# BananaFalls/LDPC-NeuralNetwork-Decoder

Hardware: AMD Instinct MI355X
Metric: codewords/s at fixed SNR (BG2, 10 iters) (higher is better)
Workload: dtype f32

## Files before the change

ldpc-neuralnetwork-decoder_amd/csrc/flood_dev.hpp:

```cpp
#pragma once
#include <algorithm>
#include <cmath>
#include <cstdint>
#include <cstdlib>

#include <utility>

#include "common.hpp"
#include "graph.hpp"

namespace ldpc {

constexpr int kPartRow = 8;
constexpr int ES_P1 = 3, ES_P2 = 4;

struct EsWs {
    uint64_t *words;
    uint32_t *valid;
    int nvw;
    uint64_t *cand;
    int32_t *twg;
    int32_t *ctl;
    uint64_t *staged;
};
// ... 95 lines not shown
typedef float f32x2 __attribute__((ext_vector_type(2)));

struct MinSumStats {
    int nz = 0;
    bool neg = false;
    float m1 = INFINITY, m2 = INFINITY;
    int i1 = -1;
    __device__ __forceinline__ void add(int e, float x) {
        const float a = fabsf(x);
        nz += is_zero_sign(x);
        neg ^= (x < 0.0f);
        const bool lt1 = a < m1, lt2 = a < m2;
        m2 = lt1 ? m1 : (lt2 ? a : m2);
        i1 = lt1 ? e : i1;
        m1 = lt1 ? a : m1;
    }
    __device__ __forceinline__ float c2v(int e, float x, float alpha) const {
        const float m = (e == i1) ? m2 : m1;
        const int zex = nz - (int)is_zero_sign(x);
        const float s = zex > 0 ? 0.0f : ((neg ^ (x < 0.0f)) ? -1.0f : 1.0f);
        return s * (alpha * m);
    }
};

template <int DC, int CAP>
__device__ __forceinline__ uint32_t sign_parity_n(const float (&v)[CAP]) {
    static_assert(DC <= CAP, "row longer than its buffer");
    uint32_t p = __float_as_uint(v[0]);
#pragma unroll
    for (int e = 1; e + 1 < DC; e += 2)
        asm("v_bitop3_b32 %0, %1, %2, %3 bitop3:0x96" : "=v"(p) : "v"(p), "v"(v[e]), "v"(v[e + 1]));
    if constexpr (DC % 2 == 0) p ^= __float_as_uint(v[DC - 1]);
    return p;
}

__device__ __forceinline__ float opaque_sf(float v) {
    asm volatile("" : "+s"(v));
    return v;
}
__device__ __forceinline__ uint32_t opaque_vu(uint32_t v) {
    asm volatile("" : "+v"(v));
    return v;
}
__device__ __forceinline__ float opaque_vf(float v) {
    asm volatile("" : "+v"(v));
    return v;
}
__device__ __forceinline__ void two_min_step(float &m1, float &m2, float x, float ninf) {
    m2 = __builtin_amdgcn_fmed3f(m1, fabsf(x), m2);
    m1 = __builtin_amdgcn_fmed3f(m1, fabsf(x), ninf);
}

__device__ __forceinline__ float vmin(float a, float b) { return __builtin_elementwise_minimum(a, b); }
__device__ __forceinline__ float vmax(float a, float b) { return __builtin_elementwise_maximum(a, b); }
template <int DC, int CAP>
__device__ __forceinline__ void two_smallest(const float (&v)[CAP], float &m1, float &m2, float ninf) {
    static_assert(DC <= CAP, "row longer than its buffer");
    if constexpr (DC == 1) {
        m1 = fabsf(v[0]);
    } else if constexpr (DC == 2) {
        m1 = vmin(fabsf(v[0]), fabsf(v[1]));
        m2 = vmax(fabsf(v[0]), fabsf(v[1]));
    } else {
        m1 = vmin(vmin(fabsf(v[0]), fabsf(v[1])), fabsf(v[2]));
        m2 = __builtin_amdgcn_fmed3f(fabsf(v[0]), fabsf(v[1]), fabsf(v[2]));
        constexpr int NT = (DC - 3) / 3;
        sfor<NT>([&](auto q) {
            constexpr int B0 = 3 + 3 * decltype(q)::value;
            const float a = fabsf(v[B0]), b = fabsf(v[B0 + 1]), c = fabsf(v[B0 + 2]);
            const float t1 = vmin(vmin(a, b), c), t2 = __builtin_amdgcn_fmed3f(a, b, c);
            m2 = vmin(vmin(vmax(m1, t1), m2), t2);
            m1 = vmin(m1, t1);
        });
        sfor<DC - 3 - 3 * NT>([&](auto q) { two_min_step(m1, m2, v[3 + 3 * NT + decltype(q)::value], ninf); });
    }
}

__device__ __forceinline__ uint64_t cmp_eq_abs(float x, float m) {
    uint64_t k;
    asm volatile("v_cmp_eq_f32_e64 %0, |%1|, %2" : "=s"(k) : "v"(x), "v"(m));
    return k;
}
__device__ __forceinline__ uint32_t cndmask(uint32_t if0, uint32_t if1, uint64_t k) {
    uint32_t r;
    asm volatile("v_cndmask_b32_e64 %0, %1, %2, %3" : "=v"(r) : "v"(if0), "v"(if1), "s"(k));
    return r;
}

struct MinSumFast {
    float m1 = INFINITY, m2 = INFINITY;
    uint32_t par = 0;
    bool special = false;
    __device__ __forceinline__ void add(float x) {
        const float a = fabsf(x);
        special |= is_zero_sign(x);
        m2 = __builtin_amdgcn_fmed3f(m1, a, m2);
        asm("v_min_f32 %0, %1, |%2|" : "=v"(m1) : "v"(m1), "v"(x));
    }
    __device__ __forceinline__ float c2v(float x, uint32_t s1, uint32_t s2) const {
        const uint32_t sel = fabsf(x) == m1 ? s2 : s1;
        return __uint_as_float((__float_as_uint(x) & 0x80000000u) ^ sel);
    }
    __device__ __forceinline__ void sel_words(float alpha, uint32_t &s1, uint32_t &s2) const {
        const uint32_t ps = par & 0x80000000u;
        s1 = __float_as_uint(fabsf(alpha * m1)) | ps;
        s2 = __float_as_uint(fabsf(alpha * m2)) | ps;
    }
};

__device__ __forceinline__ float tanh_half(float v) {
    const float y = v * 0.5f;
    const float a = fabsf(y), z = y * y;
    float p = fmaf(-5.70498872745e-3f, z, 2.06390887954e-2f);
    p = fmaf(p, z, -5.37397155531e-2f);
    p = fmaf(p, z, 1.33314422036e-1f);
    p = fmaf(p, z, -3.33332819422e-1f);
    const float small = fmaf(p * z, a, a);
    const float e = __builtin_amdgcn_exp2f(a * 2.88539008177792681f);
    const float big = fmaf(-2.0f, __builtin_amdgcn_rcpf(e + 1.0f), 1.0f);
    return copysignf(a < 0.625f ? small : big, y);
}
__device__ __forceinline__ float two_atanh(float x) {
    const float z = x * x;
    float p = fmaf(1.81740078349e-1f, z, 8.24370301058e-2f);
    p = fmaf(p, z, 1.46691431730e-1f);
    p = fmaf(p, z, 1.99782164500e-1f);
    p = fmaf(p, z, 3.33337300303e-1f);
    const float small = 2.0f * fmaf(p * z, x, x);
    const float r = (1.0f + x) * __builtin_amdgcn_rcpf(1.0f - x);
    const float big = __builtin_amdgcn_logf(r) * 0.693147180559945309f;
    return fabsf(x) < 0.5f ? small : big;
}

struct Ctx {
    FloodTables T;
    char *lds;
    uint64_t *words;
    uint32_t *flag;
    uint32_t *redo;
    float alpha;
    int out_dtype;
    void *bits;
    bool direct_bits;
    bool ballots;
};

__device__ __forceinline__ uint64_t seg_rotl(uint64_t w, int s, int z, uint64_t rep1) {
    if (s == 0) return w;
    if (z >= 64) return (w << s) | (w >> (64 - s));
    const uint64_t low = ((1ull << (z - s)) - 1ull) * rep1;
    return ((w & low) << s) | ((w & ~low) >> (z - s));
}

__device__ __forceinline__ void ext_decision(const Ctx &C, const Lane &L, int col, int s4, float app,
                                             int &errs) {
    const int bit = app < 0.0f;
    if (C.direct_bits && L.valid) {
        int64_t fr = L.frame;
        int k4 = L.k4;
        asm volatile("" : "+v"(fr), "+v"(k4));
        put_bit(C.bits, C.out_dtype, fr * C.T.N + (col * L.z4 + ((k4 + s4) & L.zmask4)) / 4, bit);
        errs += bit;
    }
    if (C.ballots) {
        const uint64_t w = seg_rotl(__ballot(bit), s4 >> 2, C.T.Z, C.T.rep1);
        if (L.lane == 0) C.words[col] = w;
    }
}

__device__ __forceinline__ void var_decision(const Ctx &C, const Lane &L, int col, float app, int &errs) {
    const int bit = app < 0.0f;
    if (C.direct_bits && L.valid) {
        int64_t fr = L.frame;
        int k = L.k;
        asm volatile("" : "+v"(fr), "+v"(k));
        put_bit(C.bits, C.out_dtype, fr * C.T.N + (int64_t)col * L.Z() + k, bit);
        errs += bit;
    }
    if (C.ballots) {
        const uint64_t w = __ballot(bit);
        if (L.lane == 0) C.words[col] = w;
    }
}

template <int ALGO, int DC>
__device__ __forceinline__ void check_task(const Ctx &C, const Lane &L, const int32_t *prog, int &errs) {
    float v[DC];
    int32_t w[DC];
#pragma unroll
    for (int e = 0; e < DC; ++e) {
        w[e] = tab(prog, e);
        const int lo = w[e] & kLowMask, s4 = (w[e] >> kShiftBit) & 0xFF;
        v[e] = w[e] < 0 ? L.llr_at(L.col_off(lo, s4)) : lds_rd(C.lds, lo + L.lane4);
    }
    auto emit = [&](int e, float o) {
        const int lo = w[e] & kLowMask;
        if (w[e] >= 0)
            lds_wr(C.lds, lo + L.lane4, o);
        else if (C.direct_bits || C.ballots)
            ext_decision(C, L, lo, (w[e] >> kShiftBit) & 0xFF, v[e] + o, errs);
    };
    if constexpr (ALGO == LDPC_ALGO_MINSUM) {
        MinSumFast fs;
#pragma unroll
        for (int e = 0; e < DC; ++e) fs.add(v[e]);
        fs.par = sign_parity_n<DC>(v);
        if (!__any(fs.special)) {
            uint32_t s1, s2;
            fs.sel_words(C.alpha, s1, s2);
#pragma unroll
            for (int e = 0; e < DC; ++e) emit(e, fs.c2v(v[e], s1, s2));
        } else {
            MinSumStats st;
#pragma unroll
            for (int e = 0; e < DC; ++e) st.add(e, v[e]);
#pragma unroll
            for (int e = 0; e < DC; ++e) emit(e, st.c2v(e, v[e], C.alpha));
        }
    } else {
        float acc[DC];
        float P = 1.0f;
#pragma unroll
        for (int j = 0; j < DC; ++j) {
            const float t = tanh_half(v[j]);
#pragma unroll
            for (int e = 0; e < j; ++e) acc[e] = acc[e] * t;
            acc[j] = P;
            P = P * t;
        }
#pragma unroll
        for (int e = 0; e < DC; ++e) emit(e, two_atanh(acc[e]));
    }
}

template <int ALGO>
__device__ __forceinline__ void check_task_dyn(const Ctx &C, const Lane &L, const int32_t *prog, int dc,
                                               int &errs) {
    auto rd = [&](int e) -> float {
        const int32_t w = tab(prog, e);
        const int lo = w & kLowMask;
        return w < 0 ? L.llr_at(L.col_off(lo, (w >> kShiftBit) & 0xFF)) : lds_rd(C.lds, lo + L.lane4);
    };
    auto wr = [&](int e, float in, float out) {
        const int32_t w = tab(prog, e);
        const int lo = w & kLowMask;
        if (w >= 0)
            lds_wr(C.lds, lo + L.lane4, out);
        else if (C.direct_bits || C.ballots)
            ext_decision(C, L, lo, (w >> kShiftBit) & 0xFF, in + out, errs);
    };
    if constexpr (ALGO == LDPC_ALGO_MINSUM) {
        MinSumStats st;
        for (int e = 0; e < dc; ++e) st.add(e, rd(e));
        for (int e = 0; e < dc; ++e) {
            const float x = rd(e);
            wr(e, x, st.c2v(e, x, C.alpha));
        }
    } else {
        float P = 1.0f;
        for (int e = 0; e < dc; ++e) {
            const float x = rd(e);
            float rr = P;
            for (int q = e + 1; q < dc; ++q) rr = rr * tanh_half(rd(q));
            const float t = tanh_half(x);
            wr(e, x, two_atanh(rr));
            P = P * t;
        }
    }
}

template <int DV>
__device__ __forceinline__ void var_task(const Ctx &C, const Lane &L, const int32_t *prog, int col, bool write,
                                         int &errs) {
    float P = L.llr_at(col * L.z4 + L.k4);
    if constexpr (DV > 0) {
        float acc[DV];
        int off[DV];
#pragma unroll
        for (int j = 0; j < DV; ++j) {
            const int32_t w = tab(prog, j);
            off[j] = (w & kLowMask) + L.vrot((w >> kShiftBit) & 0xFF);
            const float c = lds_rd(C.lds, off[j]);
#pragma unroll
            for (int e = 0; e < j; ++e) acc[e] = acc[e] + c;
            acc[j] = P;
            P = P + c;
        }
        if (write) {
#pragma unroll
            for (int e = 0; e < DV; ++e) lds_wr(C.lds, off[e], acc[e]);
        }
    }
    if (C.direct_bits || C.ballots) var_decision(C, L, col, P, errs);
}

__device__ __forceinline__ void var_task_dyn(const Ctx &C, const Lane &L, const int32_t *prog, int dv, int col,
                                             bool write, int &errs) {
    auto off = [&](int e) {
        const int32_t w = tab(prog, e);
        return (w & kLowMask) + L.vrot((w >> kShiftBit) & 0xFF);
    };
    float P = L.llr_at(col * L.z4 + L.k4);
    for (int e = 0; e < dv; ++e) {
        const int o = off(e);
        const float cp = lds_rd(C.lds, o);
        float acc = P;
        for (int q = e + 1; q < dv; ++q) acc = acc + lds_rd(C.lds, off(q));
        P = P + cp;
        if (write) lds_wr(C.lds, o, acc);
    }
    if (C.direct_bits || C.ballots) var_decision(C, L, col, P, errs);
}

#define LDPC_DC_CASES(X) X(1) X(2) X(3) X(4) X(5) X(6) X(7) X(8) X(9) X(10) X(11) X(12)
#define LDPC_DV_CASES(X) \
    X(1) X(2) X(3) X(4) X(5) X(6) X(7) X(8) X(9) X(10) X(11) X(12) X(13) X(14) X(15) X(16) \
    X(17) X(18) X(19) X(20) X(21) X(22) X(23) X(24)

template <int ALGO>
__device__ __forceinline__ void check_phase(const Ctx &C, const Lane &L, int wave, int &errs) {
    const int p1 = tab(C.T.prog_ptr, wave + 1);
    for (int pc = tab(C.T.prog_ptr, wave); pc < p1;) {
        const int dc = tab(C.T.chk_prog, pc);
        const int32_t *prog = C.T.chk_prog + pc + 1;
        switch (dc) {
            case 0: break;
#define X(n) case n: check_task<ALGO, n>(C, L, prog, errs); break;
            LDPC_DC_CASES(X)
#undef X
            default: check_task_dyn<ALGO>(C, L, prog, dc, errs); break;
        }
        pc += 1 + dc;
    }
}

// ... 17 lines not shown

__device__ __forceinline__ void init_phase(const Ctx &C, const Lane &L, int wave) {
    const int W1 = C.T.W + 1;
    const int p1 = tab(C.T.prog_ptr, W1 + wave + 1);
    for (int pc = tab(C.T.prog_ptr, W1 + wave); pc < p1;) {
        const int h = tab(C.T.var_prog, pc);
        const int dv = h & 0xFF, col = h >> 8;
        const float x = L.llr_at(col * L.z4 + L.k4);
        for (int e = 0; e < dv; ++e) {
            const int32_t w = tab(C.T.var_prog, pc + 1 + e);
            lds_wr(C.lds, (w & kLowMask) + L.vrot((w >> kShiftBit) & 0xFF), x);
        }
        pc += 1 + dv;
    }
}

__device__ __forceinline__ int parity_phase(const Ctx &C, const Lane &L, int wave) {
    const int W1 = C.T.W + 1;
    const int p1 = tab(C.T.prog_ptr, 2 * W1 + wave + 1);
    int inv = 0;
    for (int pc = tab(C.T.prog_ptr, 2 * W1 + wave); pc < p1;) {
        const int dc = tab(C.T.par_prog, pc);
        int p = 0;
        for (int e = 0; e < dc; ++e) {
            const int32_t w = tab(C.T.par_prog, pc + 1 + e);
            const int col = w & kLowMask, s = w >> kShiftBit;
            p ^= (int)((C.words[col] >> (L.f * L.Z() + ((L.k + s) & (L.Z() - 1)))) & 1ull);
        }
        inv |= p;
        pc += 1 + dc;
    }
    return inv;
}

__device__ __forceinline__ uint64_t frame_valid_mask(uint64_t invalid_lanes, int Z, int FG) {
    const uint64_t seg = Z >= 64 ? ~0ull : ((1ull << Z) - 1ull);
    uint64_t m = 0;
    for (int f = 0; f < FG; ++f)
        if (((invalid_lanes >> (f * Z)) & seg) == 0) m |= 1ull << f;
    return m;
}

__device__ __forceinline__ void emit_from_words(const Ctx &C, const Lane &L, const uint64_t *words, uint64_t mask,
                                                int wave, int &errs) {
    if (!(L.valid && ((mask >> L.f) & 1ull))) return;
    const int W1 = C.T.W + 1;
    for (int i = tab(C.T.prog_ptr, 3 * W1 + wave); i < tab(C.T.prog_ptr, 3 * W1 + wave + 1); ++i) {
        const int col = tab(C.T.bw_task, i);
        const int bit = (int)((words[col] >> L.lane) & 1ull);
        put_bit(C.bits, C.out_dtype, L.frame * C.T.N + (int64_t)col * L.Z() + L.k, bit);
        errs += bit;
    }
}

__device__ __forceinline__ void reduce_counters(void *lds, const Lane &L, int errs, int my_iters, int nf,
                                                int Z, uint32_t *row) {
    uint32_t *u = reinterpret_cast<uint32_t *>(lds);
    const int nt = blockDim.x;
    __syncthreads();
    u[threadIdx.x] = (uint32_t)errs;
    u[nt + threadIdx.x] = (uint32_t)my_iters;
    __syncthreads();
    if (threadIdx.x < 64) {
        const int f = threadIdx.x;
        uint32_t be = 0, fe = 0, fr = 0, it = 0, itmax = 0;
        if (f < nf) {
            for (int w = 0; w < nt / 64; ++w)
                for (int k = 0; k < Z; ++k) be += u[w * 64 + f * Z + k];
            fe = be > 0;
            fr = 1;
            it = u[nt + f * Z];
            itmax = it;
        }
        for (int off = 32; off > 0; off >>= 1) {
            be += __shfl_xor(be, off, 64);
            fe += __shfl_xor(fe, off, 64);
            fr += __shfl_xor(fr, off, 64);
            it += __shfl_xor(it, off, 64);
            itmax = max(itmax, (uint32_t)__shfl_xor(itmax, off, 64));
        }
        if (f == 0) {
            row[0] = be;
            row[1] = fe;
            row[2] = fr;
            row[3] = it;
            row[4] = itmax;
        }
    }
}

__device__ __forceinline__ Lane make_lane(const FloodTables &T, const float *llr, int64_t B, int group) {
    Lane L;
    L.group = group;
    L.lane = threadIdx.x & 63;
    const int lz = __builtin_ctz((unsigned)T.Z);
    L.f = L.lane >> lz;
    L.k = L.lane & (T.Z - 1);
    L.lane4 = 4 * L.lane;
    L.fz4 = 4 * (L.f << lz);
    L.k4 = 4 * L.k;
    L.z4 = 4 * T.Z;
    L.zmask4 = 4 * T.Z - 1;
    L.frame = (int64_t)group * T.FG + L.f;
    L.valid = L.frame < B;
    L.llr_row = reinterpret_cast<const char *>(llr ? llr + (L.valid ? L.frame : 0) * (int64_t)T.N : nullptr);
    return L;
}
__device__ __forceinline__ Lane make_lane(const FloodTables &T, const float *llr, int64_t B) {
    return make_lane(T, llr, B, (int)blockIdx.x);
}


template <int ES, class Body>
__device__ __forceinline__ void flood_drive(Body &body, Ctx &C, const Lane &L, int64_t B, int max_iter,
                                            const Outs &O, const EsWs &W) {
    const int tid = threadIdx.x;
    const int wave = __builtin_amdgcn_readfirstlane(tid >> 6);
    const int FG = C.T.FG, Nb = C.T.Nb, Z = C.T.Z;
    const int nf = (int)min<int64_t>((int64_t)FG, B - (int64_t)L.group * FG);
    const uint64_t exist = nf >= 64 ? ~0ull : ((1ull << nf) - 1ull);
    int errs = 0;
    if constexpr (ES == LDPC_ES_BATCH) {
        if (__builtin_amdgcn_readfirstlane(W.ctl[2]) == 0) return;
    }
    if constexpr (ES == ES_P2) {
        const int T = __builtin_amdgcn_readfirstlane(W.ctl[0]);
        if (__builtin_amdgcn_readfirstlane(W.twg[L.group]) == T) {
            emit_from_words(C, L, W.cand + (int64_t)L.group * Nb, exist, wave, errs);
            if (O.iters_out && L.valid && L.k == 0) O.iters_out[L.frame] = T;
            reduce_counters(C.lds, L, errs, T, nf, Z, O.partials + (int64_t)L.group * kPartRow);
            return;
        }
        max_iter = T;
    }
    if (tid == 0) *C.flag = 0;
    __syncthreads();
    body.init(C, L);
    __syncthreads();
#ifdef LDPC_TIMELINE
    uint64_t *tl = (O.timeline && blockIdx.x < (unsigned)kTlWgs && L.lane == 0)
                       ? O.timeline + ((int64_t)blockIdx.x * 4 + wave) * kTlPer : nullptr;
    auto mark = [&](int k) {
        const uint64_t t = tl_now();
        if (tl && k < kTlPer - kTlTail) tl[k] = t;
    };
#else
    auto mark = [](int) {};
#endif
    mark(0);

    int my_iters = max_iter;
    uint64_t done = 0;
    constexpr bool kEvery = ES == LDPC_ES_BATCH || ES == LDPC_ES_FRAME || ES == ES_P1;
    for (int it = 0; it < max_iter; ++it) {
        const bool last = it == max_iter - 1;
        C.direct_bits = (ES == LDPC_ES_OFF || ES == ES_P2) && last;
        C.ballots = ES == LDPC_ES_BATCH || ES == LDPC_ES_FRAME || ES == ES_P1 || (ES == ES_P2 && last);
        if constexpr (Body::kBail) {
            if (__builtin_amdgcn_readfirstlane(*C.flag) != 0) {
                if (tid == 0) C.redo[1 + atomicAdd(C.redo, 1u)] = (uint32_t)L.group;
                return;
            }
        }
        if (kEvery || last)
            body.template check<true>(C, L, errs);
        else
            body.template check<false>(C, L, errs);
        mark(1 + 4 * it);
        __syncthreads();
        mark(2 + 4 * it);
        if (C.ballots && tid == 0) C.words[Nb] = 0;
        if (last)
            body.template var<true, false>(C, L, errs);
        else if (kEvery)
            body.template var<true, true>(C, L, errs);
        else
            body.template var<false, true>(C, L, errs);
        mark(3 + 4 * it);
        __syncthreads();
        mark(4 + 4 * it);
        if (C.ballots) {
            const uint64_t m = __ballot(body.parity(C, L));
            if (L.lane == 0 && m) atomicOr((unsigned long long *)&C.words[Nb], (unsigned long long)m);
            __syncthreads();
            const uint64_t vmask = frame_valid_mask(C.words[Nb], Z, FG) & exist;
            bool stop = false;
            if constexpr (ES == LDPC_ES_BATCH) {
                if (L.valid && L.k == 0 && ((vmask >> L.f) & 1ull))
                    W.valid[L.frame * W.nvw + (it >> 5)] |= 1u << (it & 31);
                uint64_t *dst = W.words + ((int64_t)L.group * max_iter + it) * Nb;
                for (int c = tid; c < Nb; c += blockDim.x) dst[c] = C.words[c];
            } else if constexpr (ES == LDPC_ES_FRAME) {
                const uint64_t newly = vmask & ~done;
                if (newly) {
                    emit_from_words(C, L, C.words, newly, wave, errs);
                    if ((newly >> L.f) & 1ull) my_iters = it + 1;
                    if (O.iters_out && L.valid && L.k == 0 && ((newly >> L.f) & 1ull)) O.iters_out[L.frame] = it + 1;
                    done |= newly;
                }
                stop = done == exist;
            } else if constexpr (ES == ES_P1) {
                stop = vmask == exist || last;
                if (stop) {
                    uint64_t *dst = W.cand + (int64_t)L.group * Nb;
                    for (int c = tid; c < Nb; c += blockDim.x) dst[c] = C.words[c];
                    if (tid == 0) {
                        W.twg[L.group] = it + 1;
                        atomicMax(&W.ctl[0], it + 1);
                    }
                }
            } else if constexpr (ES == ES_P2) {
                if (vmask != exist && tid == 0) atomicOr(&W.ctl[1], 1);
            }
            __syncthreads();
            if (stop) break;
        }
    }
    if constexpr (ES == LDPC_ES_FRAME) {
        const uint64_t rest = exist & ~done;
        if (rest) {
            emit_from_words(C, L, C.words, rest, wave, errs);
            if (O.iters_out && L.valid && L.k == 0 && ((rest >> L.f) & 1ull)) O.iters_out[L.frame] = max_iter;
        }
    }
    if constexpr (ES == LDPC_ES_OFF || ES == ES_P2) {
        if (O.iters_out && L.valid && L.k == 0) O.iters_out[L.frame] = max_iter;
    }
    if constexpr (ES == LDPC_ES_OFF || ES == LDPC_ES_FRAME) {
        if (O.partials) reduce_counters(C.lds, L, errs, my_iters, nf, Z, O.partials + (int64_t)L.group * kPartRow);
    }
    if constexpr (ES == ES_P2) reduce_counters(C.lds, L, errs, max_iter, nf, Z, O.partials + (int64_t)L.group * kPartRow);
}

template <int ALGO>
struct GenericBody {
    static constexpr bool kBail = false;
    int wave;
    __device__ __forceinline__ void init(Ctx &C, const Lane &L) { init_phase(C, L, wave); }
    template <bool DEC>
    __device__ __forceinline__ void check(const Ctx &C, const Lane &L, int &errs) { check_phase<ALGO>(C, L, wave, errs); }
    template <bool DEC, bool WRITE>
    __device__ __forceinline__ void var(const Ctx &C, const Lane &L, int &errs) {
        var_phase(C, L, wave, WRITE, errs);
    }
    __device__ __forceinline__ int parity(const Ctx &C, const Lane &L) { return parity_phase(C, L, wave); }
};

__device__ __forceinline__ void init_ctx(Ctx &C, const FloodTables &T, char *lds, float alpha, int out_dtype,
                                         void *bits) {
    C.T = T;
    C.lds = lds;
    C.flag = reinterpret_cast<uint32_t *>(lds + (size_t)T.nslots * 256);
    C.words = reinterpret_cast<uint64_t *>(lds + (size_t)T.nslots * 256 + 8);
    C.alpha = alpha;
    C.out_dtype = out_dtype;
    C.bits = bits;
    C.direct_bits = false;
    C.ballots = false;
    C.redo = nullptr;
}

}

template <int ALGO, int ES>
__global__ __launch_bounds__(512) void flood_kernel(FloodTables T, const float *__restrict__ llr, int64_t B,
                                                    int max_iter, float alpha, int out_dtype,
                                                    void *__restrict__ bits, Outs O, EsWs W) {
    extern __shared__ __attribute__((aligned(16))) char lds[];
    const Lane L = make_lane(T, llr, B);
    Ctx C;
    init_ctx(C, T, lds, alpha, out_dtype, bits);
    GenericBody<ALGO> body{__builtin_amdgcn_readfirstlane((int)threadIdx.x >> 6)};
    flood_drive<ES>(body, C, L, B, max_iter, O, W);
}

}
```

ldpc-neuralnetwork-decoder_amd/csrc/flood_fixed.hpp:

```cpp
#pragma once
#include "flood_host.hpp"
#include "gen/fixed_codes.hpp"

namespace ldpc {
namespace {

constexpr bool reg_edges(int algo) { return algo == LDPC_ALGO_MINSUM; }

#ifndef LDPC_SLOW_REG_EDGES
#define LDPC_SLOW_REG_EDGES 16
#endif
#ifndef LDPC_SLOW_REG_EDGES_OFF
#define LDPC_SLOW_REG_EDGES_OFF 6
#endif
constexpr int kAllRegEdges = 1 << 20;
template <int ES, bool BAIL>
constexpr int reg_edge_cap() {
    return BAIL ? kAllRegEdges : (ES == LDPC_ES_OFF ? LDPC_SLOW_REG_EDGES_OFF : LDPC_SLOW_REG_EDGES);
}

template <class G, int WV, int CAP, bool REG>
struct FxPlan {
    static constexpr int R0 = REG ? G::RE_CHK_PTR[WV] : G::CHK_PTR[WV];
    static constexpr int NR = (REG ? G::RE_CHK_PTR[WV + 1] : G::CHK_PTR[WV + 1]) - R0;
    static constexpr int NREG = !REG ? 0 : (G::RE_NREG[WV] < CAP ? G::RE_NREG[WV] : CAP);
    static constexpr int chk_row(int i) { return REG ? G::RE_CHK_ROWS[R0 + i] : G::CHK_ROWS[R0 + i]; }
    static constexpr int row_shift(int e) { return REG ? G::RE_ROW_SHIFT[e] : G::ROW_SHIFT[e]; }
    static constexpr int col_shift(int j) { return REG ? G::RE_COL_SHIFT[j] : G::COL_SHIFT[j]; }
    static constexpr int row_reg(int e) { return REG && G::RE_ROW_REG[e] < CAP ? G::RE_ROW_REG[e] : -1; }
    static constexpr int col_reg(int j) { return REG && G::RE_COL_REG[j] < CAP ? G::RE_COL_REG[j] : -1; }
    static constexpr int C0 = G::VT_COL_PTR[WV], NC = G::VT_COL_PTR[WV + 1] - C0;
    static constexpr int T0 = G::VT_PTR[WV], NT = G::VT_PTR[WV + 1] - T0;
    static constexpr int col_index(int col) {
        for (int i = 0; i < NC; ++i)
            if (G::VT_COLS[C0 + i] == col) return i;
        return -1;
    }
    struct Tab {
        int nsh = 0, next = 0, maxdc = 1, maxdv = 1;
        int shv[64] = {};
        int shidx[64] = {};
        int ext_before[64] = {};
    };
    static constexpr int inv_shift(int s) { return (G::Z - s) % G::Z; }
    static constexpr Tab make() {
        Tab t{};
        for (int i = 0; i < 64; ++i) t.shidx[i] = -1;
        auto use = [&t](int s) {
            if (t.shidx[s] < 0) {
                t.shidx[s] = t.nsh;
                t.shv[t.nsh++] = s;
            }
        };
        for (int i = 0; i < NC; ++i) {
            const int c = G::VT_COLS[C0 + i];
            const int dv = G::COL_PTR[c + 1] - G::COL_PTR[c];
            if (dv > t.maxdv) t.maxdv = dv;
            for (int j = G::COL_PTR[c]; j < G::COL_PTR[c + 1]; ++j)
                if (col_reg(j) < 0) use(col_shift(j));
        }
        for (int i = 0; i < NR; ++i) {
            const int R = chk_row(i);
            t.ext_before[i] = t.next;
            const int dc = G::ROW_PTR[R + 1] - G::ROW_PTR[R];
            if (dc > t.maxdc) t.maxdc = dc;
            for (int e = G::ROW_PTR[R]; e < G::ROW_PTR[R + 1]; ++e) {
                if (G::ROW_SLOT[e] < 0)
                    ++t.next;
                else if (row_reg(e) < 0)
                    use(inv_shift(row_shift(e)));
            }
        }
        return t;
    }
    static constexpr Tab T = make();
    static constexpr int ext_index(int i, int e) {
        const int R = chk_row(i);
        int x = T.ext_before[i];
        for (int q = 0; q < e; ++q)
            if (G::ROW_SLOT[G::ROW_PTR[R] + q] < 0) ++x;
        return x;
    }
};

constexpr int kVarPipe = 24;

#ifndef LDPC_DIRECT_DC
#define LDPC_DIRECT_DC 6
#endif
constexpr int kDirectDc = LDPC_DIRECT_DC;
static_assert(kDirectDc >= 0 && kDirectDc <= 6, "direct_row is written out for degrees 2 .. 6");

__device__ __forceinline__ uint32_t xor3(uint32_t a, uint32_t b, uint32_t c) { return __builtin_amdgcn_bitop3_b32(a, b, c, 0x96); }

template <int DC, int E, int CAP>
__device__ __forceinline__ float direct_row(const float (&v)[CAP], const float (&pr)[3], float als, float alv, uint32_t sgn) {
    static_assert(DC >= 2 && DC <= 6 && E < DC && DC <= CAP, "direct form: degrees 2 .. 6");
    constexpr int A = E == 0 ? 1 : 0, B = E <= 1 ? 2 : 1, Cc = E <= 2 ? 3 : 2;
    auto bits = [&](int e) { return __float_as_uint(v[e]); };
    if constexpr (DC == 2) {
        return __uint_as_float(__builtin_amdgcn_bitop3_b32(__float_as_uint(alv * fabsf(v[A])), bits(A), sgn, 0x78));
    } else if constexpr (DC == 3) {
        const float m = vmin(fabsf(v[A]), fabsf(v[B]));
        return __uint_as_float(__builtin_amdgcn_bitop3_b32(__float_as_uint(alv * m), bits(A) ^ bits(B), sgn, 0x78));
    } else if constexpr (DC == 4) {
        const float m = vmin(vmin(fabsf(v[A]), fabsf(v[B])), fabsf(v[Cc]));
        return __uint_as_float(__builtin_amdgcn_bitop3_b32(__float_as_uint(alv * m), xor3(bits(A), bits(B), bits(Cc)), sgn, 0x78));
    } else {
        constexpr int PE = E / 2;
        float m;
        if constexpr (DC == 5 && E == 4)
            m = vmin(pr[0], pr[1]);
        else if constexpr (DC == 5)
            m = vmin(vmin(fabsf(v[E ^ 1]), pr[1 - PE]), fabsf(v[4]));
        else
            m = vmin(vmin(fabsf(v[E ^ 1]), pr[(PE + 1) % 3]), pr[(PE + 2) % 3]);
        return __uint_as_float(__builtin_amdgcn_bitop3_b32(__float_as_uint(als * m), bits(E), sgn, 0x78));
    }
}

template <class G, int ALGO, int WV, bool BAIL, int CAP, bool REG>
struct FixedBody {
    static_assert(!BAIL || ALGO == LDPC_ALGO_MINSUM, "only min-sum has a fast and an exact check update");
    static constexpr bool kBail = BAIL;
    using P = FxPlan<G, WV, CAP, REG>;
    static constexpr int ZM4 = 4 * G::Z - 1;
    static constexpr int NEXT = P::T.next > 0 ? P::T.next : 1;
    static constexpr int NCOL = P::NC > 0 ? P::NC : 1;
    static constexpr int NSH = P::T.nsh > 0 ? P::T.nsh : 1;
    static constexpr int MAXDC = P::T.maxdc, MAXDV = P::T.maxdv;
    static constexpr int NRG = P::NREG > 0 ? P::NREG : 1;
    float ext[NEXT];
    float cllr[NCOL];
    uint32_t rot[NSH];
    float msg[NRG];

    __device__ __forceinline__ void init(Ctx &C, const Lane &L) {
        bool nan = false;
        sfor<P::NR>([&](auto i) {
            constexpr int I = decltype(i)::value, R = P::chk_row(I);
            constexpr int P0 = G::ROW_PTR[R], DC = G::ROW_PTR[R + 1] - P0;
            sfor<DC>([&](auto e) {
                constexpr int E = decltype(e)::value;
                if constexpr (G::ROW_SLOT[P0 + E] < 0) {
                    constexpr int X = P::ext_index(I, E), COL = G::ROW_COL[P0 + E], S4 = 4 * P::row_shift(P0 + E);
                    ext[X] = L.llr_at(COL * 4 * G::Z + ((L.k4 + S4) & ZM4));
                    nan |= !(fabsf(ext[X]) < INFINITY);
                }
            });
        });
        sfor<P::T.nsh>([&](auto j) {
            constexpr int J = decltype(j)::value, SH = P::T.shv[J];
            const uint32_t base = (uint32_t)(uintptr_t)C.lds;
            if constexpr (SH == 0)
                rot[J] = opaque_vu(base + L.lane4);
            else
                rot[J] = opaque_vu(base + L.fz4 + ((L.k4 + (4 * G::Z - 4 * SH)) & ZM4));
        });
        addtid_begin(C.lds);
        sfor<P::NC>([&](auto i) {
            constexpr int I = decltype(i)::value, COL = G::VT_COLS[P::C0 + I];
            constexpr int P0 = G::COL_PTR[COL], DV = G::COL_PTR[COL + 1] - P0;
            cllr[I] = L.llr_at(COL * 4 * G::Z + L.k4);
            nan |= !(fabsf(cllr[I]) < INFINITY);
            sfor<DV>([&](auto jj) {
                constexpr int J = P0 + decltype(jj)::value;
                if constexpr (P::col_reg(J) >= 0)
                    msg[P::col_reg(J)] = cllr[I];
                else
                    lds_wr_tid<G::COL_SLOT[J] * 256>(cllr[I]);
            });
        });
        addtid_end();
        if (__any(nan) && L.lane == 0) *C.flag = 1;
    }

    template <int I>
    __device__ __forceinline__ void load_row(const Ctx &C, const Lane &L, float (&v)[MAXDC]) const {
        constexpr int R = P::chk_row(I), P0 = G::ROW_PTR[R], DC = G::ROW_PTR[R + 1] - P0;
        sfor<DC>([&](auto e) {
            constexpr int E = decltype(e)::value, SL = G::ROW_SLOT[P0 + E];
            if constexpr (P::row_reg(P0 + E) >= 0)
                v[E] = msg[P::row_reg(P0 + E)];
            else if constexpr (SL >= 0)
                v[E] = lds_rd_abs<SL * 256>(rot[P::T.shidx[P::inv_shift(P::row_shift(P0 + E))]]);
            else
                v[E] = ext[P::ext_index(I, E)];
        });
    }

    template <int I, bool DEC, bool SLOW = false>
    __device__ __forceinline__ void row(const Ctx &C, const Lane &L, const float (&v)[MAXDC], int &errs, float ninf, float pinf, uint32_t sgn, float alv) {
        constexpr int R = P::chk_row(I), P0 = G::ROW_PTR[R], DC = G::ROW_PTR[R + 1] - P0;
        auto needed = [](int e) constexpr { return DEC || G::ROW_SLOT[P0 + e] >= 0; };
        auto emit = [&](auto e, float o) {
            constexpr int E = decltype(e)::value, SL = G::ROW_SLOT[P0 + E];
            if constexpr (P::row_reg(P0 + E) >= 0) {
                msg[P::row_reg(P0 + E)] = o;
            } else if constexpr (SL >= 0) {
                lds_wr_tid<SL * 256>(o);
            } else if constexpr (DEC) {
                if (C.direct_bits || C.ballots)
                    ext_decision(C, L, G::ROW_COL[P0 + E], 4 * P::row_shift(P0 + E), v[E] + o, errs);
            }
        };
        if constexpr (ALGO == LDPC_ALGO_MINSUM && !SLOW && DC >= 2 && DC <= kDirectDc) {
            float pr[3] = {};
            float als = alv;
            if constexpr (DC >= 5) {
                sfor<DC / 2>([&](auto j) {
                    constexpr int J = decltype(j)::value;
                    pr[J] = vmin(fabsf(v[2 * J]), fabsf(v[2 * J + 1]));
                });
                uint32_t par = xor3(__float_as_uint(v[0]), __float_as_uint(v[1]), __float_as_uint(v[2]));
                if constexpr (DC == 5)
                    par = xor3(par, __float_as_uint(v[3]), __float_as_uint(v[4]));
                else
                    par = xor3(par, __float_as_uint(v[3]), __float_as_uint(v[4])) ^ __float_as_uint(v[5]);
                als = __uint_as_float(__builtin_amdgcn_bitop3_b32(__float_as_uint(alv), par, sgn, 0x78));
            }
            sfor<DC>([&](auto e) {
                constexpr int E = decltype(e)::value;
                if constexpr (needed(E)) emit(e, direct_row<DC, E>(v, pr, als, alv, sgn));
            });
        } else if constexpr (ALGO == LDPC_ALGO_MINSUM) {
            float m1 = fabsf(v[0]), m2 = pinf;
            two_smallest<DC>(v, m1, m2, ninf);
            if (!SLOW) {
                const uint32_t par = sign_parity_n<DC>(v) & sgn;
                const uint32_t s1 = __float_as_uint(alv * m1) ^ par, s2 = __float_as_uint(alv * m2) ^ par;
                uint64_t mk[DC];
                uint32_t sel[DC];
                sfor<DC + 3>([&](auto q) {
                    constexpr int Q = decltype(q)::value;
                    if constexpr (Q < DC && needed(Q)) mk[Q] = cmp_eq_abs(v[Q], m1);
                    if constexpr (Q >= 3 && needed(Q - 3)) sel[Q - 3] = cndmask(s1, s2, mk[Q - 3]);
                });
                sfor<DC>([&](auto e) {
                    constexpr int E = decltype(e)::value;
                    if constexpr (needed(E))
                        emit(e, __uint_as_float(__builtin_amdgcn_bitop3_b32(sel[E], __float_as_uint(v[E]), sgn, 0x78)));
                });
            } else {
                MinSumStats st;
                sfor<DC>([&](auto e) { st.add(decltype(e)::value, v[decltype(e)::value]); });
                sfor<DC>([&](auto e) { emit(e, st.c2v(decltype(e)::value, v[decltype(e)::value], C.alpha)); });
            }
        } else {
            float acc[DC];
            float Pp = 1.0f;
            sfor<DC>([&](auto jj) {
                constexpr int J = decltype(jj)::value;
                const float t = tanh_half(v[J]);
                sfor<J>([&](auto e) { acc[decltype(e)::value] = acc[decltype(e)::value] * t; });
                acc[J] = Pp;
                Pp = Pp * t;
            });
            sfor<DC>([&](auto e) { emit(e, two_atanh(acc[decltype(e)::value])); });
        }
    }

    template <bool DEC>
    __device__ __forceinline__ void check(const Ctx &C, const Lane &L, int &errs) {
        if constexpr (ALGO == LDPC_ALGO_MINSUM && !BAIL) {
            if (__builtin_amdgcn_readfirstlane(*C.flag) != 0)
                rows<DEC, true>(C, L, errs);
            else
                rows<DEC, false>(C, L, errs);
            return;
        }
        rows<DEC, false>(C, L, errs);
    }

    template <bool DEC, bool SLOW>
    __device__ __forceinline__ void rows(const Ctx &C, const Lane &L, int &errs) {
        float va[MAXDC], vb[MAXDC];
        addtid_begin(C.lds);
        const float ninf = opaque_sf(-INFINITY), pinf = opaque_sf(INFINITY);
        const uint32_t sgn = opaque_vu(0x80000000u);
        const float alv = opaque_vf(C.alpha);
        load_row<0>(C, L, va);
        sfor<P::NR>([&](auto i) {
            constexpr int I = decltype(i)::value;
            if constexpr (I % 2 == 0) {
                if constexpr (I + 1 < P::NR) load_row<I + 1>(C, L, vb);
                row<I, DEC, SLOW>(C, L, va, errs, ninf, pinf, sgn, alv);
            } else {
                if constexpr (I + 1 < P::NR) load_row<I + 1>(C, L, va);
                row<I, DEC, SLOW>(C, L, vb, errs, ninf, pinf, sgn, alv);
            }
        });
        addtid_end();
    }

    template <int TK>
    struct Task {
        static constexpr int X = P::T0 + TK;
        static constexpr int CA = G::VT_A[X], CB = G::VT_B[X];
        static constexpr int PA = G::COL_PTR[CA], DA = G::COL_PTR[CA + 1] - PA;
        static constexpr int PB = CB >= 0 ? G::COL_PTR[CB] : 0, DB = CB >= 0 ? G::COL_PTR[CB + 1] - PB : 0;
        static_assert(DB <= DA, "pair tasks: A is the longer column");
        static constexpr int IA = P::col_index(CA), IB = CB >= 0 ? P::col_index(CB) : 0;
        static constexpr int NMSG = DA + DB;
    };
    struct TaskIn {
        f32x2 cp[MAXDV];
        float cs[MAXDV];
    };

    template <int X>
    __device__ __forceinline__ float c2v_in() const {
        if constexpr (P::col_reg(X) >= 0)
            return msg[P::col_reg(X)];
        else
            return lds_rd_abs<G::COL_SLOT[X] * 256>(rot[P::T.shidx[P::col_shift(X)]]);
    }
    template <int X>
    __device__ __forceinline__ void v2c_out(float o) {
        if constexpr (P::col_reg(X) >= 0)
            msg[P::col_reg(X)] = o;
        else
            lds_wr_tid<G::COL_SLOT[X] * 256>(o);
    }

    template <int TK>
    __device__ __forceinline__ void load_task(const Ctx &C, TaskIn &in) const {
        using K = Task<TK>;
        sfor<K::DA>([&](auto jj) {
            constexpr int J = decltype(jj)::value;
            if constexpr (J < K::DB) {
                in.cp[J].x = c2v_in<K::PA + J>();
                in.cp[J].y = c2v_in<K::PB + J>();
            } else {
                in.cs[J] = c2v_in<K::PA + J>();
            }
        });
    }

    template <int TK, bool DEC, bool WRITE>
    __device__ __forceinline__ void task(const Ctx &C, const Lane &L, const TaskIn &in, int &errs, bool &bad) {
        using K = Task<TK>;
        constexpr int DA = K::DA, DB = K::DB;
        f32x2 P2;
        float PA = cllr[K::IA];
        if constexpr (DB > 0) {
            P2.x = cllr[K::IA];
            P2.y = cllr[K::IB];
        }
        f32x2 acc2[DB > 0 ? DB : 1];
        float accA[DA];
        sfor<DA>([&](auto jj) {
            constexpr int J = decltype(jj)::value;
            if constexpr (J < DB) {
                sfor<J>([&](auto e) {
                    constexpr int E = decltype(e)::value;
                    acc2[E] = acc2[E] + in.cp[J];
                });
                acc2[J] = P2;
                P2 = P2 + in.cp[J];
                if constexpr (J == DB - 1) PA = P2.x;
            } else {
                sfor<J>([&](auto e) {
                    constexpr int E = decltype(e)::value;
                    if constexpr (E < DB)
                        acc2[E].x = acc2[E].x + in.cs[J];
                    else
                        accA[E] = accA[E] + in.cs[J];
                });
                accA[J] = PA;
                PA = PA + in.cs[J];
            }
        });
        if constexpr (WRITE) {
            sfor<DA>([&](auto e) {
                constexpr int E = decltype(e)::value;
                if constexpr (E < DB) {
                    v2c_out<K::PA + E>(acc2[E].x);
                    v2c_out<K::PB + E>(acc2[E].y);
                } else {
                    v2c_out<K::PA + E>(accA[E]);
                }
            });
        }
        if constexpr (ALGO == LDPC_ALGO_MINSUM) bad |= !(fabsf(PA) < INFINITY);
        if constexpr (DEC) {
            if (C.direct_bits || C.ballots) var_decision(C, L, K::CA, PA, errs);
        }
        if constexpr (DB > 0) {
            if constexpr (ALGO == LDPC_ALGO_MINSUM) bad |= !(fabsf(P2.y) < INFINITY);
            if constexpr (DEC) {
                if (C.direct_bits || C.ballots) var_decision(C, L, K::CB, P2.y, errs);
            }
        }
    }

    template <bool DEC, bool WRITE>
    __device__ __forceinline__ void var(const Ctx &C, const Lane &L, int &errs) {
        bool bad = false;
        if constexpr (P::NT > 0) {
            TaskIn ta, tb;
            if constexpr (WRITE) addtid_begin(C.lds);
            load_task<0>(C, ta);
            sfor<P::NT>([&](auto i) {
                constexpr int I = decltype(i)::value;
                constexpr bool more = I + 1 < P::NT;
                constexpr bool ahead = more && Task<I>::NMSG + Task<(more ? I + 1 : I)>::NMSG <= kVarPipe;
                if constexpr (I % 2 == 0) {
                    if constexpr (ahead) load_task<I + 1>(C, tb);
                    task<I, DEC, WRITE>(C, L, ta, errs, bad);
                    if constexpr (more && !ahead) load_task<(more ? I + 1 : I)>(C, tb);
                } else {
                    if constexpr (ahead) load_task<I + 1>(C, ta);
                    task<I, DEC, WRITE>(C, L, tb, errs, bad);
                    if constexpr (more && !ahead) load_task<(more ? I + 1 : I)>(C, ta);
                }
            });
            if constexpr (WRITE) addtid_end();
        }
        if constexpr (ALGO == LDPC_ALGO_MINSUM) {
            if (__any(bad) && L.lane == 0) *C.flag = 1;
        }
    }

    __device__ __forceinline__ int parity(const Ctx &C, const Lane &L) const {
        int inv = 0;
        int f = L.f, k = L.k;
        asm volatile("" : "+v"(f), "+v"(k));
        sfor<P::NR>([&](auto i) {
            constexpr int R = P::chk_row(decltype(i)::value);
            constexpr int P0 = G::ROW_PTR[R], DC = G::ROW_PTR[R + 1] - P0;
            int p = 0;
            sfor<DC>([&](auto e) {
                constexpr int E = decltype(e)::value;
                constexpr int COL = G::ROW_COL[P0 + E], S = P::row_shift(P0 + E);
                p ^= (int)(C.words[COL] >> (f * G::Z + ((k + S) & (G::Z - 1))));
            });
            inv |= p;
        });
        return inv & 1;
    }
};

template <class G, class F>
__device__ __forceinline__ void fx_by_wave(int wave, F &&f) {
    static_assert(G::W == 4, "fixed schedules are generated for 4 waves");
    switch (wave) {
        case 0: f(ic<0>{}); break;
        case 1: f(ic<1>{}); break;
        case 2: f(ic<2>{}); break;
        default: f(ic<3>{}); break;
    }
}

}

template <class G, int ALGO, int ES, bool BAIL = false>
__global__ __launch_bounds__(256, ES == LDPC_ES_OFF ? 4 : 3) void flood_fixed_kernel(FloodTables T, const float *__restrict__ llr,
                                                          int64_t B, int max_iter, float alpha, int out_dtype,
                                                          void *__restrict__ bits, Outs O, EsWs W, uint32_t *redo) {
    static_assert(!BAIL || ES == LDPC_ES_OFF || ES == LDPC_ES_FRAME, "the batch-stop passes share state across workgroups");
    extern __shared__ __attribute__((aligned(16))) char lds[];
#ifdef LDPC_TIMELINE
    const uint64_t t_in = tl_now();
#endif
    FloodTables Tc = T;
    Tc.Z = G::Z, Tc.FG = 64 / G::Z, Tc.Mb = G::Mb, Tc.Nb = G::Nb, Tc.N = G::N, Tc.nslots = G::NSLOTS, Tc.W = G::W;
    static_assert(G::Z < 64 && 64 % G::Z == 0, "rep1 below: a 1 at the bottom of every Z-bit segment");
    Tc.rep1 = ~0ull / ((1ull << G::Z) - 1ull);
    const Lane L = make_lane(Tc, llr, B);
    Ctx C;
    init_ctx(C, Tc, lds, alpha, out_dtype, bits);
    if constexpr (BAIL) C.redo = redo;
    fx_by_wave<G>(__builtin_amdgcn_readfirstlane((int)threadIdx.x >> 6), [&](auto wv) {
        FixedBody<G, ALGO, decltype(wv)::value, BAIL, reg_edge_cap<ES, BAIL>(), reg_edges(ALGO)> body;
        flood_drive<ES>(body, C, L, B, max_iter, O, W);
#ifdef LDPC_TIMELINE
        if constexpr (ES == LDPC_ES_OFF) tl_bracket(O.timeline, decltype(wv)::value, t_in);
#endif
    });
}

template <int ALGO>
int launch_fixed(const FloodCall &c, int es, size_t lds, const Outs &O, const EsWs &W, uint32_t *redo) {
    auto pick = [&](auto code) -> const void * {
        using G = decltype(code);
        if constexpr (ALGO == LDPC_ALGO_MINSUM) {
            if (redo && es == LDPC_ES_OFF) return reinterpret_cast<const void *>(flood_fixed_kernel<G, ALGO, LDPC_ES_OFF, true>);
            if (redo && es == LDPC_ES_FRAME) return reinterpret_cast<const void *>(flood_fixed_kernel<G, ALGO, LDPC_ES_FRAME, true>);
        }
        if (redo) return nullptr;
        switch (es) {
            case LDPC_ES_OFF: return reinterpret_cast<const void *>(flood_fixed_kernel<G, ALGO, LDPC_ES_OFF>);
            case LDPC_ES_FRAME: return reinterpret_cast<const void *>(flood_fixed_kernel<G, ALGO, LDPC_ES_FRAME>);
            case LDPC_ES_BATCH: return reinterpret_cast<const void *>(flood_fixed_kernel<G, ALGO, LDPC_ES_BATCH>);
            case ES_P1: return reinterpret_cast<const void *>(flood_fixed_kernel<G, ALGO, ES_P1>);
            case ES_P2: return reinterpret_cast<const void *>(flood_fixed_kernel<G, ALGO, ES_P2>);
            default: return nullptr;
        }
    };
    const int id = c.g->fixed_id;
    const void *kern = id == 1 ? pick(fixed::BG2_Z4{}) : (id == 2 ? pick(fixed::BG2_Z32{}) : nullptr);
    if (!kern) return fail(LDPC_EINVAL, "no fixed kernel for this code / stopping mode");
    LDPC_HIP(hipFuncSetAttribute(kern, hipFuncAttributeMaxDynamicSharedMemorySize, (int)lds));
    FloodCall a = c;
    FloodTables t = c.g->ft;
    Outs o = O;
    EsWs w = W;
    void *args[] = {&t, &a.llr, &a.B, &a.max_iter, &a.alpha, &a.out_dtype, &a.bits, &o, &w, &redo};
    const int64_t nwg = (c.B + c.g->FG - 1) / c.g->FG;
    LDPC_HIP(hipLaunchKernel(kern, dim3((unsigned)nwg), dim3(64 * c.g->ft.W), args, lds, c.s));
    return LDPC_OK;
}

}
```

Baseline: 71.58 million.

## Peel last decoder iteration and specialize hard-decision stores by output dtype

Restructures the iteration loop into a lambda so that, for fixed-plan bodies without per-iteration early stopping, the first max_iter-1 iterations compile without any decision or ballot code and the final iteration is a separate, fully specialized instance. The final iteration's bit stores go through a DecOut helper with compile-time column and shift offsets and output element size, replacing the generic runtime put_bit address arithmetic. The aim is to remove runtime branches and register pressure from the hot non-final iterations and to make the last-iteration stores cheaper. In exchange the kernel gets larger from extra template instantiations, and the new helper assumes Z is a power of two dividing N.

```diff
diff --git a/ldpc-neuralnetwork-decoder_amd/csrc/flood_dev.hpp b/ldpc-neuralnetwork-decoder_amd/csrc/flood_dev.hpp
--- a/ldpc-neuralnetwork-decoder_amd/csrc/flood_dev.hpp
+++ b/ldpc-neuralnetwork-decoder_amd/csrc/flood_dev.hpp
@@ -271,6 +271,15 @@
     return ((w & low) << s) | ((w & ~low) >> (z - s));
 }
 
+__device__ __forceinline__ void var_ballot(const Ctx &C, const Lane &L, int col, int bit) {
+    const uint64_t w = __ballot(bit);
+    if (L.lane == 0) C.words[col] = w;
+}
+__device__ __forceinline__ void ext_ballot(const Ctx &C, const Lane &L, int col, int s4, int bit) {
+    const uint64_t w = seg_rotl(__ballot(bit), s4 >> 2, C.T.Z, C.T.rep1);
+    if (L.lane == 0) C.words[col] = w;
+}
+
 __device__ __forceinline__ void ext_decision(const Ctx &C, const Lane &L, int col, int s4, float app,
                                              int &errs) {
     const int bit = app < 0.0f;
@@ -281,10 +290,7 @@
         put_bit(C.bits, C.out_dtype, fr * C.T.N + (col * L.z4 + ((k4 + s4) & L.zmask4)) / 4, bit);
         errs += bit;
     }
-    if (C.ballots) {
-        const uint64_t w = seg_rotl(__ballot(bit), s4 >> 2, C.T.Z, C.T.rep1);
-        if (L.lane == 0) C.words[col] = w;
-    }
+    if (C.ballots) ext_ballot(C, L, col, s4, bit);
 }
 
 __device__ __forceinline__ void var_decision(const Ctx &C, const Lane &L, int col, float app, int &errs) {
@@ -296,10 +302,7 @@
         put_bit(C.bits, C.out_dtype, fr * C.T.N + (int64_t)col * L.Z() + k, bit);
         errs += bit;
     }
-    if (C.ballots) {
-        const uint64_t w = __ballot(bit);
-        if (L.lane == 0) C.words[col] = w;
-    }
+    if (C.ballots) var_ballot(C, L, col, bit);
 }
 
 template <int ALGO, int DC>
@@ -623,39 +626,56 @@
     int my_iters = max_iter;
     uint64_t done = 0;
     constexpr bool kEvery = ES == LDPC_ES_BATCH || ES == LDPC_ES_FRAME || ES == ES_P1;
-    for (int it = 0; it < max_iter; ++it) {
-        const bool last = it == max_iter - 1;
-        C.direct_bits = (ES == LDPC_ES_OFF || ES == ES_P2) && last;
-        C.ballots = ES == LDPC_ES_BATCH || ES == LDPC_ES_FRAME || ES == ES_P1 || (ES == ES_P2 && last);
+    constexpr int kGoOn = 0, kStop = 1, kLeft = 2;
+    constexpr bool kPeel = !kEvery && Body::kPeel;
+    auto iteration = [&](auto when, int it) __attribute__((always_inline)) -> int {
+        constexpr int WHEN = decltype(when)::value;
+        static_assert(kPeel ? WHEN < 2 : WHEN == 2, "the last iteration is peeled or it is not");
+        const bool last = WHEN == 2 ? it == max_iter - 1 : WHEN == 1;
+        constexpr bool DIRECT = WHEN == 1;
+        C.direct_bits = !kEvery && last;
+        C.ballots = kEvery || (ES == ES_P2 && last);
         if constexpr (Body::kBail) {
-            if (__builtin_amdgcn_readfirstlane(*C.flag) != 0) {
+            if (__builtin_expect(__builtin_amdgcn_readfirstlane(*C.flag) != 0, 0)) {
                 if (tid == 0) C.redo[1 + atomicAdd(C.redo, 1u)] = (uint32_t)L.group;
-                return;
+                return kLeft;
             }
         }
-        if (kEvery || last)
-            body.template check<true>(C, L, errs);
-        else
-            body.template check<false>(C, L, errs);
+        if constexpr (WHEN == 0) {
+            body.template check<false, false>(C, L, errs);
+        } else if constexpr (WHEN == 1 || kEvery) {
+            body.template check<true, DIRECT>(C, L, errs);
+        } else {
+            if (last)
+                body.template check<true, false>(C, L, errs);
+            else
+                body.template check<false, false>(C, L, errs);
+        }
         mark(1 + 4 * it);
         __syncthreads();
         mark(2 + 4 * it);
         if (C.ballots && tid == 0) C.words[Nb] = 0;
-        if (last)
-            body.template var<true, false>(C, L, errs);
-        else if (kEvery)
-            body.template var<true, true>(C, L, errs);
-        else
-            body.template var<false, true>(C, L, errs);
+        if constexpr (WHEN == 0) {
+            body.template var<false, true, false>(C, L, errs);
+        } else if constexpr (WHEN == 1) {
+            body.template var<true, false, DIRECT>(C, L, errs);
+        } else {
+            if (last)
+                body.template var<true, false, false>(C, L, errs);
+            else if (kEvery)
+                body.template var<true, true, false>(C, L, errs);
+            else
+                body.template var<false, true, false>(C, L, errs);
+        }
         mark(3 + 4 * it);
         __syncthreads();
         mark(4 + 4 * it);
+        bool stop = false;
         if (C.ballots) {
             const uint64_t m = __ballot(body.parity(C, L));
             if (L.lane == 0 && m) atomicOr((unsigned long long *)&C.words[Nb], (unsigned long long)m);
             __syncthreads();
             const uint64_t vmask = frame_valid_mask(C.words[Nb], Z, FG) & exist;
-            bool stop = false;
             if constexpr (ES == LDPC_ES_BATCH) {
                 if (L.valid && L.k == 0 && ((vmask >> L.f) & 1ull))
                     W.valid[L.frame * W.nvw + (it >> 5)] |= 1u << (it & 31);
@@ -684,8 +704,19 @@
                 if (vmask != exist && tid == 0) atomicOr(&W.ctl[1], 1);
             }
             __syncthreads();
-            if (stop) break;
-        }
+        }
+        return stop ? kStop : kGoOn;
+    };
+    if constexpr (!kPeel) {
+        for (int it = 0; it < max_iter; ++it) {
+            const int r = iteration(ic<2>{}, it);
+            if (r == kLeft) return;
+            if (r == kStop) break;
+        }
+    } else {
+        for (int it = 0; it < max_iter - 1; ++it)
+            if (iteration(ic<0>{}, it) == kLeft) return;
+        if (max_iter > 0 && iteration(ic<1>{}, max_iter - 1) == kLeft) return;
     }
     if constexpr (ES == LDPC_ES_FRAME) {
         const uint64_t rest = exist & ~done;
@@ -706,11 +737,12 @@
 template <int ALGO>
 struct GenericBody {
     static constexpr bool kBail = false;
+    static constexpr bool kPeel = false;
     int wave;
     __device__ __forceinline__ void init(Ctx &C, const Lane &L) { init_phase(C, L, wave); }
-    template <bool DEC>
+    template <bool DEC, bool DIRECT>
     __device__ __forceinline__ void check(const Ctx &C, const Lane &L, int &errs) { check_phase<ALGO>(C, L, wave, errs); }
-    template <bool DEC, bool WRITE>
+    template <bool DEC, bool WRITE, bool DIRECT>
     __device__ __forceinline__ void var(const Ctx &C, const Lane &L, int &errs) {
         var_phase(C, L, wave, WRITE, errs);
     }
diff --git a/ldpc-neuralnetwork-decoder_amd/csrc/flood_fixed.hpp b/ldpc-neuralnetwork-decoder_amd/csrc/flood_fixed.hpp
--- a/ldpc-neuralnetwork-decoder_amd/csrc/flood_fixed.hpp
+++ b/ldpc-neuralnetwork-decoder_amd/csrc/flood_fixed.hpp
@@ -119,10 +119,58 @@
     }
 }
 
+constexpr int kOutAny = 2;
+template <class G, int OUT>
+struct DecOut {
+    static_assert(OUT == LDPC_OUT_U8 || OUT == LDPC_OUT_F32 || OUT == kOutAny, "one form per output type");
+    static_assert(G::N % G::Z == 0 && (G::Z & (G::Z - 1)) == 0, "rotated(): row | position");
+    char *base;
+    uint32_t row;
+    uint32_t own;
+    uint32_t kb;
+    uint32_t any;
+    bool valid;
+    __device__ __forceinline__ uint32_t size() const {
+        if constexpr (OUT == kOutAny)
+            return any;
+        else
+            return OUT == LDPC_OUT_F32 ? 4u : 1u;
+    }
+    __device__ __forceinline__ DecOut(const Ctx &C, const Lane &L) {
+        any = C.out_dtype == LDPC_OUT_F32 ? 4u : 1u;
+        base = static_cast<char *>(C.bits) + (int64_t)L.group * (64 / G::Z) * G::N * size();
+        row = (uint32_t)L.f * (G::N * size());
+        kb = (uint32_t)L.k * size();
+        own = row + kb;
+        valid = L.valid;
+    }
+    __device__ __forceinline__ void put(uint32_t off, int bit, int &errs) const {
+        if (valid) {
+            if (size() == 4u)
+                *reinterpret_cast<float *>(base + off) = (float)bit;
+            else
+                *reinterpret_cast<uint8_t *>(base + off) = (uint8_t)bit;
+        }
+        errs += bit;
+    }
+    template <int COL>
+    __device__ __forceinline__ void col(int bit, int &errs) const { put(own + COL * G::Z * size(), bit, errs); }
+    template <int COL, int S>
+    __device__ __forceinline__ void rotated(int bit, int &errs) const {
+        put((row | ((kb + S * size()) & (G::Z * size() - 1))) + COL * G::Z * size(), bit, errs);
+    }
+};
+struct NoOut {
+    __device__ __forceinline__ NoOut(const Ctx &, const Lane &) {}
+};
+template <class G, int OUT>
+using DecOutFor = std::conditional_t<OUT < 0, NoOut, DecOut<G, OUT>>;
+
 template <class G, int ALGO, int WV, bool BAIL, int CAP, bool REG>
 struct FixedBody {
     static_assert(!BAIL || ALGO == LDPC_ALGO_MINSUM, "only min-sum has a fast and an exact check update");
     static constexpr bool kBail = BAIL;
+    static constexpr bool kPeel = true;
     using P = FxPlan<G, WV, CAP, REG>;
     static constexpr int ZM4 = 4 * G::Z - 1;
     static constexpr int NEXT = P::T.next > 0 ? P::T.next : 1;
@@ -189,8 +237,8 @@
         });
     }
 
-    template <int I, bool DEC, bool SLOW = false>
-    __device__ __forceinline__ void row(const Ctx &C, const Lane &L, const float (&v)[MAXDC], int &errs, float ninf, float pinf, uint32_t sgn, float alv) {
+    template <int I, bool DEC, bool SLOW, int OUT>
+    __device__ __forceinline__ void row(const Ctx &C, const Lane &L, const DecOutFor<G, OUT> &D, const float (&v)[MAXDC], int &errs, float ninf, float pinf, uint32_t sgn, float alv) {
         constexpr int R = P::chk_row(I), P0 = G::ROW_PTR[R], DC = G::ROW_PTR[R + 1] - P0;
         auto needed = [](int e) constexpr { return DEC || G::ROW_SLOT[P0 + e] >= 0; };
         auto emit = [&](auto e, float o) {
@@ -200,8 +248,10 @@
             } else if constexpr (SL >= 0) {
                 lds_wr_tid<SL * 256>(o);
             } else if constexpr (DEC) {
-                if (C.direct_bits || C.ballots)
-                    ext_decision(C, L, G::ROW_COL[P0 + E], 4 * P::row_shift(P0 + E), v[E] + o, errs);
+                constexpr int COL = G::ROW_COL[P0 + E], S = P::row_shift(P0 + E);
+                const int bit = v[E] + o < 0.0f;
+                if constexpr (OUT >= 0) D.template rotated<COL, S>(bit, errs);
+                if (C.ballots) ext_ballot(C, L, COL, 4 * S, bit);
             }
         };
         if constexpr (ALGO == LDPC_ALGO_MINSUM && !SLOW && DC >= 2 && DC <= kDirectDc) {
@@ -260,21 +310,27 @@
         }
     }
 
-    template <bool DEC>
+    template <bool DEC, bool DIRECT>
     __device__ __forceinline__ void check(const Ctx &C, const Lane &L, int &errs) {
+        static_assert(DEC || !DIRECT, "stores need decisions");
         if constexpr (ALGO == LDPC_ALGO_MINSUM && !BAIL) {
-            if (__builtin_amdgcn_readfirstlane(*C.flag) != 0)
-                rows<DEC, true>(C, L, errs);
-            else
-                rows<DEC, false>(C, L, errs);
-            return;
-        }
-        rows<DEC, false>(C, L, errs);
-    }
-
-    template <bool DEC, bool SLOW>
+            if (__builtin_amdgcn_readfirstlane(*C.flag) != 0) {
+                rows<DEC, true, (DIRECT ? kOutAny : -1)>(C, L, errs);
+                return;
+            }
+        }
+        if constexpr (!DIRECT)
+            rows<DEC, false, -1>(C, L, errs);
+        else if (C.out_dtype == LDPC_OUT_F32)
+            rows<DEC, false, LDPC_OUT_F32>(C, L, errs);
+        else
+            rows<DEC, false, LDPC_OUT_U8>(C, L, errs);
+    }
+
+    template <bool DEC, bool SLOW, int OUT>
     __device__ __forceinline__ void rows(const Ctx &C, const Lane &L, int &errs) {
         float va[MAXDC], vb[MAXDC];
+        const DecOutFor<G, OUT> D(C, L);
         addtid_begin(C.lds);
         const float ninf = opaque_sf(-INFINITY), pinf = opaque_sf(INFINITY);
         const uint32_t sgn = opaque_vu(0x80000000u);
@@ -284,10 +340,10 @@
             constexpr int I = decltype(i)::value;
             if constexpr (I % 2 == 0) {
                 if constexpr (I + 1 < P::NR) load_row<I + 1>(C, L, vb);
-                row<I, DEC, SLOW>(C, L, va, errs, ninf, pinf, sgn, alv);
+                row<I, DEC, SLOW, OUT>(C, L, D, va, errs, ninf, pinf, sgn, alv);
             } else {
                 if constexpr (I + 1 < P::NR) load_row<I + 1>(C, L, va);
-                row<I, DEC, SLOW>(C, L, vb, errs, ninf, pinf, sgn, alv);
+                row<I, DEC, SLOW, OUT>(C, L, D, vb, errs, ninf, pinf, sgn, alv);
             }
         });
         addtid_end();
@@ -337,8 +393,8 @@
         });
     }
 
-    template <int TK, bool DEC, bool WRITE>
-    __device__ __forceinline__ void task(const Ctx &C, const Lane &L, const TaskIn &in, int &errs, bool &bad) {
+    template <int TK, bool DEC, bool WRITE, int OUT>
+    __device__ __forceinline__ void task(const Ctx &C, const Lane &L, const DecOutFor<G, OUT> &D, const TaskIn &in, int &errs, bool &bad) {
         using K = Task<TK>;
         constexpr int DA = K::DA, DB = K::DB;
         f32x2 P2;
@@ -382,22 +438,35 @@
                 }
             });
         }
+        auto decide = [&](auto col, float app) {
+            constexpr int COL = decltype(col)::value;
+            const int bit = app < 0.0f;
+            if constexpr (OUT >= 0) D.template col<COL>(bit, errs);
+            if (C.ballots) var_ballot(C, L, COL, bit);
+        };
         if constexpr (ALGO == LDPC_ALGO_MINSUM) bad |= !(fabsf(PA) < INFINITY);
-        if constexpr (DEC) {
-            if (C.direct_bits || C.ballots) var_decision(C, L, K::CA, PA, errs);
-        }
+        if constexpr (DEC) decide(ic<K::CA>{}, PA);
         if constexpr (DB > 0) {
             if constexpr (ALGO == LDPC_ALGO_MINSUM) bad |= !(fabsf(P2.y) < INFINITY);
-            if constexpr (DEC) {
-                if (C.direct_bits || C.ballots) var_decision(C, L, K::CB, P2.y, errs);
-            }
-        }
-    }
-
-    template <bool DEC, bool WRITE>
+            if constexpr (DEC) decide(ic<K::CB>{}, P2.y);
+        }
+    }
+
+    template <bool DEC, bool WRITE, bool DIRECT>
     __device__ __forceinline__ void var(const Ctx &C, const Lane &L, int &errs) {
+        static_assert(DEC || !DIRECT, "stores need decisions");
+        if constexpr (!DIRECT)
+            var_as<DEC, WRITE, -1>(C, L, errs);
+        else if (C.out_dtype == LDPC_OUT_F32)
+            var_as<DEC, WRITE, LDPC_OUT_F32>(C, L, errs);
+        else
+            var_as<DEC, WRITE, LDPC_OUT_U8>(C, L, errs);
+    }
+    template <bool DEC, bool WRITE, int OUT>
+    __device__ __forceinline__ void var_as(const Ctx &C, const Lane &L, int &errs) {
         bool bad = false;
         if constexpr (P::NT > 0) {
+            const DecOutFor<G, OUT> D(C, L);
             TaskIn ta, tb;
             if constexpr (WRITE) addtid_begin(C.lds);
             load_task<0>(C, ta);
@@ -407,11 +476,11 @@
                 constexpr bool ahead = more && Task<I>::NMSG + Task<(more ? I + 1 : I)>::NMSG <= kVarPipe;
                 if constexpr (I % 2 == 0) {
                     if constexpr (ahead) load_task<I + 1>(C, tb);
-                    task<I, DEC, WRITE>(C, L, ta, errs, bad);
+                    task<I, DEC, WRITE, OUT>(C, L, D, ta, errs, bad);
                     if constexpr (more && !ahead) load_task<(more ? I + 1 : I)>(C, tb);
                 } else {
                     if constexpr (ahead) load_task<I + 1>(C, ta);
-                    task<I, DEC, WRITE>(C, L, tb, errs, bad);
+                    task<I, DEC, WRITE, OUT>(C, L, D, tb, errs, bad);
                     if constexpr (more && !ahead) load_task<(more ? I + 1 : I)>(C, ta);
                 }
             });
```

New measurement: 74.43 million, median of 6. 4.0% higher.
